# nerficg-project/nerficg

Measured on NVIDIA B200. Metric: nerf_train_rays_per_s, higher is better.
Workload: dtype fp16 operands, fp32 accumulate (fp32 sampling/compositing/optimizer)

## Files before the change

include/nerf_b200.h:

```cpp
#ifndef NERF_B200_H
#define NERF_B200_H

#include <stddef.h>
#include <stdint.h>

#ifdef __cplusplus
extern "C" {
#endif

#define NERF_ABI_VERSION 1

#define NERF_N_PARAM_TENSORS 24
#define NERF_TILE 128

int nerf_abi_version(void);
const char* nerf_last_error(void);
int nerf_device_check(int device);

int nerf_param_layout(int64_t* offsets , int64_t* sizes , int64_t* total);

int nerf_sample_stratified(float* z, const float* u, int n_rays, int n_samples, float near_plane, float far_plane,
                           void* stream);

int nerf_sample_importance(float* z_merged, float* z_fine, const float* z_coarse, const float* w_coarse, const float* u,
                           int n_rays, int n_coarse, int n_fine, void* stream);

int nerf_composite_forward(float* rgb, float* depth, float* alpha, float* weights, const float* z,
                           const float* rgbsigma, const float* dirs, const float* background, int n_rays, int n_samples,
                           void* stream);

int nerf_composite_backward(float* d_rgbsigma, const float* z, const float* rgbsigma, const float* dirs,
                            const float* background, const float* g_rgb, const float* g_depth, const float* g_alpha,
                            int n_rays, int n_samples, int relu_mask, float grad_scale, void* stream);

size_t nerf_mlp_packed_bytes(void);
int nerf_mlp_pack(void* packed, const float* params, int with_backward, void* stream);

size_t nerf_mlp_stash_bytes(int64_t n_samples);
int nerf_mlp_forward(float* rgbsigma, void* stash, const void* packed, const float* params, const float* origins,
                     const float* dirs, const float* viewdirs, const float* z, const float* noise, int n_rays,
                     int n_samples, void* stream);

size_t nerf_mlp_backward_workspace_bytes(int64_t n_samples);
int nerf_mlp_backward(float* grads, const float* d_rgbsigma, const float* rgbsigma, const void* stash, void* workspace,
                      const void* packed, const float* params, int n_rays, int n_samples, float grad_scale,
                      void* stream);

int nerf_mlp_backward_pipe(float* grads, const float* d_rgbsigma, const float* rgbsigma, const void* stash, void* workspace,
                           const void* packed, const float* params, int n_rays, int n_samples, float grad_scale, void* stream);
int nerf_mlp_backward_legacy(float* grads, const float* d_rgbsigma, const float* rgbsigma, const void* stash, void* workspace,
                             const void* packed, const float* params, int n_rays, int n_samples, float grad_scale, void* stream);
size_t nerf_mlp_backward_pipe_workspace_bytes(void);

int nerf_mlp_backward_dgrad(const float* d_rgbsigma, const float* rgbsigma, const void* stash, void* workspace,
                            const void* packed, const float* params, int n_rays, int n_samples, void* stream);
int nerf_mlp_backward_wgrad(float* grads, const void* stash, const void* workspace, int n_rays, int n_samples,
                            float grad_scale, void* stream);

int nerf_adam_tick(float* state, float beta1, float beta2, void* stream);
int nerf_adam_update(float* params, float* exp_avg, float* exp_avg_sq, const float* grads, const float* lr, const float* state,
                     float beta1, float beta2, float eps, int64_t n, void* stream);
int nerf_adam_update_ex(float* params, float* exp_avg, float* exp_avg_sq, float* grads, const float* lr, const float* state,
                        float beta1, float beta2, float eps, float grad_mult, int zero_grads, int64_t n, void* stream);

int nerf_loss_mse(float* loss, float* g_rgb, float* g_rgb_coarse, float* g_alpha, float* g_alpha_coarse, const float* rgb,
                  const float* rgb_coarse, const float* alpha, const float* alpha_coarse, const float* rgb_gt,
                  const float* alpha_gt, const float* background, int n_rays, float lambda_color, float lambda_alpha, void* stream);

int nerf_debug_set_timing(void* device_buffer);

int nerf_generate_rays(float* origin, float* direction, float* view_direction, const int64_t* pixel_ids, int64_t n_rays,
                       const double* c2w_host, int width, int height, double focal_x, double focal_y, double center_x,
                       double center_y, void* stream);
int nerf_gather_rays(float* origin_dst, float* direction_dst, float* view_direction_dst, float* rgb_dst, float* alpha_dst,
                     const float* origin_src, const float* direction_src, const float* view_direction_src, const float* rgb_src,
                     const float* alpha_src, const int64_t* ids, int64_t n_rays, void* stream);

int nerf_selftest_umma(float* d_out, const float* a, const float* b, int n, int k, int mode, void* stream);
int nerf_selftest_umma2(float* d_out, const float* a, const float* b, int n, int k, void* stream);
int nerf_selftest_umma2_mn(float* d_out, const float* a, const float* b, int n, int k, void* stream);
int nerf_selftest_tmem_read(unsigned long long* out, int n_warps, int mode, int iters, void* stream);

int nerf_selftest_umma2_rate(unsigned long long* out, int mn_major, int iters, void* stream);

int nerf_selftest_l2_stream(unsigned long long* out, void* window, uint32_t window_bytes, int mode, int iters, int n_ctas, void* stream);
int nerf_selftest_l2_stream_lsu(unsigned long long* out, void* window, uint32_t window_bytes, int mode, int iters, int n_ctas, int n_warps,
                                void* stream);

#ifdef __cplusplus
}
#endif
#endif
```

nerficg_b200/_lib.py:

```python
from __future__ import annotations

import ctypes
from ctypes import c_float, c_int, c_int64, c_size_t, c_void_p
from pathlib import Path

import torch

LIB_PATH = Path(__file__).resolve().parent / 'libnerf_b200.so'

_PROTOTYPES = {
    'nerf_abi_version': (c_int, []),
    'nerf_last_error': (ctypes.c_char_p, []),
    'nerf_device_check': (c_int, [c_int]),
    'nerf_param_layout': (c_int, [ctypes.POINTER(c_int64), ctypes.POINTER(c_int64), ctypes.POINTER(c_int64)]),
    'nerf_sample_stratified': (c_int, [c_void_p, c_void_p, c_int, c_int, c_float, c_float, c_void_p]),
    'nerf_sample_importance': (c_int, [c_void_p, c_void_p, c_void_p, c_void_p, c_void_p, c_int, c_int, c_int, c_void_p]),
    'nerf_composite_forward': (c_int, [c_void_p] * 8 + [c_int, c_int, c_void_p]),
    'nerf_composite_backward': (c_int, [c_void_p] * 8 + [c_int, c_int, c_int, c_float, c_void_p]),
    'nerf_mlp_packed_bytes': (c_size_t, []),
    'nerf_mlp_pack': (c_int, [c_void_p, c_void_p, c_int, c_void_p]),
    'nerf_mlp_stash_bytes': (c_size_t, [c_int64]),
    'nerf_mlp_forward': (c_int, [c_void_p] * 9 + [c_int, c_int, c_void_p]),
    'nerf_mlp_backward_workspace_bytes': (c_size_t, [c_int64]),
    'nerf_mlp_backward': (c_int, [c_void_p] * 7 + [c_int, c_int, c_float, c_void_p]),
    'nerf_mlp_backward_pipe': (c_int, [c_void_p] * 7 + [c_int, c_int, c_float, c_void_p]),
    'nerf_mlp_backward_legacy': (c_int, [c_void_p] * 7 + [c_int, c_int, c_float, c_void_p]),
    'nerf_mlp_backward_pipe_workspace_bytes': (c_size_t, []),
    'nerf_mlp_backward_dgrad': (c_int, [c_void_p] * 6 + [c_int, c_int, c_void_p]),
    'nerf_mlp_backward_wgrad': (c_int, [c_void_p] * 3 + [c_int, c_int, c_float, c_void_p]),
    'nerf_adam_tick': (c_int, [c_void_p, c_float, c_float, c_void_p]),
    'nerf_adam_update': (c_int, [c_void_p] * 6 + [c_float, c_float, c_float, c_int64, c_void_p]),
    'nerf_adam_update_ex': (c_int, [c_void_p] * 6 + [c_float, c_float, c_float, c_float, c_int, c_int64, c_void_p]),
    'nerf_generate_rays': (c_int, [c_void_p, c_void_p, c_void_p, c_void_p, c_int64, ctypes.POINTER(ctypes.c_double), c_int, c_int,
                                   ctypes.c_double, ctypes.c_double, ctypes.c_double, ctypes.c_double, c_void_p]),
    'nerf_gather_rays': (c_int, [c_void_p] * 11 + [c_int64, c_void_p]),
    'nerf_loss_mse': (c_int, [c_void_p] * 12 + [c_int, c_float, c_float, c_void_p]),
    'nerf_debug_set_timing': (c_int, [c_void_p]),
    'nerf_selftest_umma': (c_int, [c_void_p, c_void_p, c_void_p, c_int, c_int, c_int, c_void_p]),
    'nerf_selftest_umma2': (c_int, [c_void_p, c_void_p, c_void_p, c_int, c_int, c_void_p]),
    'nerf_selftest_umma2_mn': (c_int, [c_void_p, c_void_p, c_void_p, c_int, c_int, c_void_p]),
    'nerf_selftest_tmem_read': (c_int, [c_void_p, c_int, c_int, c_int, c_void_p]),
    'nerf_selftest_umma2_rate': (c_int, [c_void_p, c_int, c_int, c_void_p]),
    'nerf_selftest_l2_stream': (c_int, [c_void_p, c_void_p, ctypes.c_uint32, c_int, c_int, c_int, c_void_p]),
    'nerf_selftest_l2_stream_lsu': (c_int, [c_void_p, c_void_p, ctypes.c_uint32, c_int, c_int, c_int, c_int, c_void_p]),
}

EXPORTED_SYMBOLS = tuple(_PROTOTYPES)
_lib = None


class NativeLibraryError(RuntimeError):
    """The CUDA extension is missing, stale or running on an unsupported device."""


def load() -> ctypes.CDLL:
    global _lib
    if _lib is not None:
        return _lib
    if not LIB_PATH.exists():
        raise NativeLibraryError(
            f'{LIB_PATH} not found: build it with `python nerficg_b200/csrc/build.py` '
            '(there is no CPU or PyTorch fallback for the NeRF hot path)')
    lib = ctypes.CDLL(str(LIB_PATH))
    for name, (res, args) in _PROTOTYPES.items():
        try:
            fn = getattr(lib, name)
        except AttributeError as e:
            raise NativeLibraryError(f'{LIB_PATH} does not export {name}; rebuild the extension') from e
        fn.restype = res
        fn.argtypes = args
    if lib.nerf_abi_version() != 1:
        raise NativeLibraryError('ABI version mismatch; rebuild the extension')
    _lib = lib
    return lib


def last_error() -> str:
    return load().nerf_last_error().decode()


def check(rc: int, what: str) -> None:
    if rc != 0:
        raise NativeLibraryError(f'{what} failed ({rc}): {last_error()}')


_checked_devices: set[int] = set()


def require_device(t: torch.Tensor) -> None:
    if not t.is_cuda:
        raise NativeLibraryError('nerficg_b200 kernels need CUDA tensors on a B200 (sm_100); there is no CPU path')
    idx = t.device.index if t.device.index is not None else torch.cuda.current_device()
    if idx not in _checked_devices:
        check(load().nerf_device_check(idx), 'nerf_device_check')
        _checked_devices.add(idx)


def ptr(t: torch.Tensor | None) -> int | None:
    return None if t is None else t.data_ptr()


def stream_ptr() -> int:
    return torch.cuda.current_stream().cuda_stream


def param_layout() -> tuple[list[int], list[int], int]:
    off = (c_int64 * 24)()
    size = (c_int64 * 24)()
    total = c_int64()
    check(load().nerf_param_layout(off, size, ctypes.byref(total)), 'nerf_param_layout')
    return list(off), list(size), total.value
```

nerficg_b200/csrc/mlp_wgrad.cu:

```cuda
#include "common.cuh"
#include "mlp_layout.cuh"
#include "tc.cuh"
#include "../../include/nerf_b200.h"

namespace nerf {
using namespace tc;

namespace wg {
constexpr int kThreads = 256;
constexpr int kMaxStages = 8;
constexpr uint32_t kHalfPanel = 8192;
constexpr uint32_t kRingBytes = 24 * kHalfPanel;
constexpr uint32_t kOffBars = kRingBytes;
constexpr uint32_t kSmemBytes = kOffBars + 256 + 1024;
constexpr int kNumJobs = 13;

struct Seg {
  int16_t buf;
  int16_t region;
  int16_t panels;
  int16_t valid;
  int32_t out_col;
};
struct Job {
  Seg a;
  Seg b[2];
  int64_t w_off;
  int32_t ld;
  int64_t bias_off;
  int32_t head;
  int32_t ctas;
};

using L = ParamLayout;
constexpr Seg seg(int buf, int region, int panels, int valid, int out_col) { return Seg{(int16_t)buf, (int16_t)region, (int16_t)panels, (int16_t)valid, out_col}; }
constexpr Seg none() { return Seg{0, 0, 0, 0, 0}; }
constexpr int gl(int l) { return kGradL7 + (7 - l); }
constexpr int hx(int l) { return kStashH0 + l; }

__constant__ Job c_jobs[kNumJobs] = {
    {seg(0, gl(1), 4, 256, 0), {seg(1, hx(0), 4, 256, 0), none()}, L::hidden_w(1), 256, L::hidden_b(1), 0, 13},
    {seg(0, gl(2), 4, 256, 0), {seg(1, hx(1), 4, 256, 0), none()}, L::hidden_w(2), 256, L::hidden_b(2), 0, 13},
    {seg(0, gl(3), 4, 256, 0), {seg(1, hx(2), 4, 256, 0), none()}, L::hidden_w(3), 256, L::hidden_b(3), 0, 13},
    {seg(0, gl(4), 4, 256, 0), {seg(1, hx(3), 4, 256, 0), none()}, L::hidden_w(4), 256, L::hidden_b(4), 0, 13},
    {seg(0, gl(5), 4, 256, 0), {seg(1, hx(4), 4, 256, 0), none()}, L::kW5, 319, L::kB5, 0, 13},
    {seg(0, gl(6), 4, 256, 0), {seg(1, hx(5), 4, 256, 0), none()}, L::hidden_w(6), 256, L::hidden_b(6), 0, 13},
    {seg(0, gl(7), 4, 256, 0), {seg(1, hx(6), 4, 256, 0), none()}, L::hidden_w(7), 256, L::hidden_b(7), 0, 13},
    {seg(0, kGradF, 4, 256, 0), {seg(1, hx(7), 4, 256, 0), none()}, L::kWF, 256, L::kBF, 0, 13},
    {seg(0, gl(0), 4, 256, 0), {seg(1, kStashEnc, 1, 63, 0), none()}, L::kW0, 63, L::kB0, 0, 9},
    {seg(0, gl(5), 4, 256, 0), {seg(1, kStashEnc, 1, 63, 256), none()}, L::kW5, 319, -1, 0, 8},
    {seg(0, kGradC0, 2, 128, 0), {seg(1, kStashF, 4, 256, 0), seg(1, kStashDir, 1, 27, 256)}, L::kWC0, 283, L::kBC0, 0, 12},
    {seg(1, kStashG, 2, 128, 0), {seg(0, kGradHead, 1, 4, 0), none()}, L::kWC1, 128, L::kBC1, 1, 6},
    {seg(1, hx(7), 4, 256, 0), {seg(0, kGradHead, 1, 4, 0), none()}, L::kWS, 256, L::kBS, 2, 9},
};
constexpr int kNumResidualJobs = 4;
__constant__ Job c_jobs_res[kNumResidualJobs] = {
    {seg(0, gl(0), 4, 256, 0), {seg(1, kStashEnc, 1, 63, 0), none()}, L::kW0, 63, L::kB0, 0, 37},
    {seg(0, gl(5), 4, 256, 0), {seg(1, kStashEnc, 1, 63, 256), none()}, L::kW5, 319, -1, 0, 37},
    {seg(0, kGradC0, 2, 128, 0), {seg(1, kStashF, 4, 256, 0), seg(1, kStashDir, 1, 27, 256)}, L::kWC0, 283, L::kBC0, 0, 52},
    {seg(1, kStashG, 2, 128, 0), {seg(0, kGradHead, 1, 4, 0), none()}, L::kWC1, 128, L::kBC1, 1, 22},
};
}

__global__ void __launch_bounds__(wg::kThreads, 1) mlp_wgrad_kernel(float* __restrict__ grads, const uint8_t* __restrict__ stash,
                                                                     const uint8_t* __restrict__ gstash, int n_tiles, float inv_scale,
                                                                     int residual) {
  using namespace wg;
  const Job* __restrict__ table = residual ? c_jobs_res : c_jobs;
  const int n_jobs = residual ? kNumResidualJobs : kNumJobs;
  int job_idx = 0, part = (int)blockIdx.x;
  while (job_idx < n_jobs && part >= table[job_idx].ctas) part -= table[job_idx++].ctas;
  if (job_idx >= n_jobs) return;
  const Job& job = table[job_idx];
  const int parts = job.ctas;
  const int tile_lo = (int)((int64_t)n_tiles * part / parts), tile_hi = (int)((int64_t)n_tiles * (part + 1) / parts);
  const int n_steps = 2 * (tile_hi - tile_lo);
  if (n_steps <= 0) return;

  extern __shared__ uint8_t smem_raw[];
  const uint32_t smem_base = (smem_u32(smem_raw) + 1023u) & ~1023u;
  const uint32_t bars = smem_base + kOffBars;
  const uint32_t bar_full = bars, bar_empty = bars + 8 * kMaxStages, bar_done = bars + 16 * kMaxStages, tmem_slot = bar_done + 8;
  const uint32_t kStageBytes = (uint32_t)(job.a.panels + job.b[0].panels + job.b[1].panels) * kHalfPanel;
  const int kStages = (int)(kRingBytes / kStageBytes) < kMaxStages ? (int)(kRingBytes / kStageBytes) : kMaxStages;
  const int warp = threadIdx.x >> 5, lane = threadIdx.x & 31;
  if (threadIdx.x == 0) {
    for (int i = 0; i < kMaxStages; ++i) {
      mbar_init(bar_full + 8 * i, 1);
      mbar_init(bar_empty + 8 * i, 2);
    }
    mbar_init(bar_done, 1);
    fence_barrier_init();
  }
  if (warp == 2) {
    tmem_alloc(tmem_slot, 512);
    tmem_relinquish();
  }
  tc_fence_before();
  __syncthreads();
  tc_fence_after();
  uint32_t tmem_base;
  asm volatile("ld.shared.b32 %0, [%1];" : "=r"(tmem_base) : "r"(tmem_slot));

  const uint64_t nt = (uint64_t)n_tiles;
  const int na = job.a.panels;
  const int nb0 = job.b[0].panels, nb1 = job.b[1].panels;
  const int halves = na / 2;
  const int n_total = 64 * (nb0 + nb1);

  auto region_ptr = [&](const Seg& s, int tile) -> const uint8_t* {
    return s.buf == 0 ? gstash + grad_region_offset(s.region, nt) + (uint64_t)tile * grad_region_tile_bytes(s.region)
                      : stash + stash_region_offset(s.region, nt) + (uint64_t)tile * stash_region_tile_bytes(s.region);
  };

  if (warp == 0) {
    if (lane == 0) {
      uint32_t stage = 0, phase = 0;
      const uint64_t stream_policy = l2_evict_first();
      const Seg* segs[3] = {&job.a, &job.b[0], &job.b[1]};
      const uint8_t* cur[3];
      uint32_t tile_stride[3];
      int panels[3];
      for (int s = 0; s < 3; ++s) {
        panels[s] = segs[s]->panels;
        cur[s] = region_ptr(*segs[s], tile_lo);
        tile_stride[s] = segs[s]->buf == 0 ? grad_region_tile_bytes(segs[s]->region) : stash_region_tile_bytes(segs[s]->region);
      }
      const uint32_t stage_bytes = (uint32_t)(na + nb0 + nb1) * kHalfPanel;
      for (int step = 0; step < n_steps; ++step) {
        const uint32_t half_off = (step & 1) * kHalfPanel;
        mbar_wait(bar_empty + 8 * stage, phase ^ 1);
        mbar_arrive_expect_tx(bar_full + 8 * stage, stage_bytes);
        uint32_t dst = smem_base + stage * kStageBytes;
#pragma unroll
        for (int s = 0; s < 3; ++s) {
          const uint8_t* src = cur[s] + half_off;
          for (int pp = 0; pp < panels[s]; ++pp) {
            bulk_g2s_hint(dst, src, kHalfPanel, bar_full + 8 * stage, stream_policy);
            dst += kHalfPanel;
            src += kPanelBytes128;
          }
          if (step & 1) cur[s] += tile_stride[s];
        }
        if (++stage == kStages) {
          stage = 0;
          phase ^= 1;
        }
      }
    }
  } else if (warp == 1) {
    if (lane == 0) {
      uint32_t stage = 0, phase = 0;
      const uint32_t idesc_b0 = make_idesc(128, 64 * nb0, kF16, kF16, 1, 1);
      const uint32_t idesc_b1 = make_idesc(128, 64, kF16, kF16, 1, 1);
      for (int step = 0; step < n_steps; ++step) {
        mbar_wait(bar_full + 8 * stage, phase);
        tc_fence_after();
        const uint32_t sa = smem_base + stage * kStageBytes;
        const uint32_t sb0 = sa + na * kHalfPanel, sb1 = sb0 + nb0 * kHalfPanel;
        for (int hm = 0; hm < halves; ++hm) {
          const uint32_t d0 = tmem_base + hm * n_total;
          for (int ks = 0; ks < 4; ++ks) {
            const uint64_t da = desc_mnmajor(sa + hm * 2 * kHalfPanel, ks, kHalfPanel);
            umma(d0, da, desc_mnmajor(sb0, ks, kHalfPanel), idesc_b0, (step | ks) != 0);
            if (nb1 > 0) umma(d0 + 64 * nb0, da, desc_mnmajor(sb1, ks, kHalfPanel), idesc_b1, (step | ks) != 0);
          }
        }
        umma_commit(bar_empty + 8 * stage);
        if (++stage == kStages) {
          stage = 0;
          phase ^= 1;
        }
      }
      umma_commit(bar_done);
    }
  } else if (warp >= 4) {
    const int t = threadIdx.x - 128;
    const bool head = job.head != 0;
    const int bias_cols = head ? 4 : (job.bias_off >= 0 ? 64 * na : 0);
    const uint32_t bias_seg_off = head ? na * kHalfPanel : 0;
    float s0 = 0.f, s1 = 0.f;
    uint32_t stage = 0, phase = 0;
    for (int step = 0; step < n_steps; ++step) {
      mbar_wait(bar_full + 8 * stage, phase);
      if (2 * t < bias_cols) {
        const int c = 2 * t;
        const uint32_t base = smem_base + stage * kStageBytes + bias_seg_off + (c >> 6) * kHalfPanel;
#pragma unroll 8
        for (int r = 0; r < 64; ++r) {
          uint32_t w;
          asm volatile("ld.shared.b32 %0, [%1];" : "=r"(w) : "r"(base + panel_offset(r, c & 63)));
          const float2 f = __half22float2(*reinterpret_cast<__half2*>(&w));
          s0 += f.x;
          s1 += f.y;
        }
      }
      named_bar_sync(1, 128);
      if (t == 0) mbar_arrive(bar_empty + 8 * stage);
      if (++stage == kStages) {
        stage = 0;
        phase ^= 1;
      }
    }
    if (2 * t < bias_cols) {
      if (!head) {
        atomicAdd(grads + job.bias_off + 2 * t, s0 * inv_scale);
        atomicAdd(grads + job.bias_off + 2 * t + 1, s1 * inv_scale);
      } else if (job.head == 1) {
        if (t == 0) {
          atomicAdd(grads + job.bias_off + 0, s0 * inv_scale);
          atomicAdd(grads + job.bias_off + 1, s1 * inv_scale);
        } else {
          atomicAdd(grads + job.bias_off + 2, s0 * inv_scale);
        }
      } else if (t == 1) {
        atomicAdd(grads + job.bias_off, s1 * inv_scale);
      }
    }
    mbar_wait(bar_done, 0);
    tc_fence_after();
    const int wq = warp & 3;
    const int n_local = wq * 32 + lane;
    for (int hm = 0; hm < halves; ++hm) {
      const int n = hm * 128 + n_local;
      const uint32_t t_row = tmem_base + hm * n_total + (static_cast<uint32_t>(wq * 32) << 16);
      if (head) {
        uint32_t v[32];
        tmem_ld32(t_row, v);
        tmem_ld_wait();
        if (job.head == 1) {
#pragma unroll
          for (int j = 0; j < 3; ++j) atomicAdd(grads + job.w_off + j * 128 + n, __uint_as_float(v[j]) * inv_scale);
        } else {
          atomicAdd(grads + job.w_off + n, __uint_as_float(v[3]) * inv_scale);
        }
        continue;
      }
      float* wrow = grads + job.w_off + (int64_t)n * job.ld;
      for (int s = 0; s < 2; ++s) {
        const Seg& sg = job.b[s];
        if (sg.panels == 0) continue;
        const int col_base = s == 0 ? 0 : 64 * nb0;
        for (int c0 = 0; c0 < 64 * sg.panels; c0 += 32) {
          if (c0 >= sg.valid) break;
          uint32_t v[32];
          tmem_ld32(t_row + col_base + c0, v);
          tmem_ld_wait();
#pragma unroll
          for (int j = 0; j < 32; ++j)
            if (c0 + j < sg.valid) atomicAdd(wrow + sg.out_col + c0 + j, __uint_as_float(v[j]) * inv_scale);
        }
      }
    }
  }
  tc_fence_before();
  __syncthreads();
  if (warp == 2) tmem_dealloc(tmem_base, 512);
}

static int launch_wgrad_table(float* grads, const uint8_t* stash, const uint8_t* gstash, int n_tiles, float inv_scale, int residual, cudaStream_t stream);

int launch_wgrad(float* grads, const uint8_t* stash, const uint8_t* gstash, int n_tiles, float inv_scale, cudaStream_t stream) {
  return launch_wgrad_table(grads, stash, gstash, n_tiles, inv_scale, 0, stream);
}
int launch_wgrad_residual(float* grads, const uint8_t* stash, const uint8_t* gstash, int n_tiles, float inv_scale, cudaStream_t stream) {
  return launch_wgrad_table(grads, stash, gstash, n_tiles, inv_scale, 1, stream);
}

static int launch_wgrad_table(float* grads, const uint8_t* stash, const uint8_t* gstash, int n_tiles, float inv_scale, int residual, cudaStream_t stream) {
  static bool attr_set_dev[64] = {};
    int dev__ = 0;
    cudaGetDevice(&dev__);
    bool& attr_set = attr_set_dev[dev__ & 63];
  if (!attr_set) {
    cudaError_t e = cudaFuncSetAttribute(mlp_wgrad_kernel, cudaFuncAttributeMaxDynamicSharedMemorySize, (int)wg::kSmemBytes);
    NERF_CHECK_ARG(e == cudaSuccess, "mlp_backward: cudaFuncSetAttribute(wgrad) failed: %s", cudaGetErrorString(e));
    attr_set = true;
  }
  mlp_wgrad_kernel<<<kNumSMs, wg::kThreads, wg::kSmemBytes, stream>>>(grads, stash, gstash, n_tiles, inv_scale, residual);
  NERF_CHECK_LAUNCH("mlp_wgrad_kernel");
  return 0;
}

}
```

nerficg_b200/csrc/tc.cuh:

```cuda
#pragma once
#include <cuda_bf16.h>
#include <cuda_fp16.h>
#include <cstdint>

namespace nerf {
namespace tc {

constexpr uint32_t kPanelCols = 64;
constexpr uint32_t kPanelRowBytes = 128;
constexpr uint32_t kAtomBytes = 1024;

__host__ __device__ __forceinline__ uint32_t panel_offset(uint32_t row, uint32_t col) {
  return (row >> 3) * kAtomBytes + (row & 7) * kPanelRowBytes + ((((col >> 3) ^ (row & 7)) & 7) << 4) + ((col & 7) << 1);
}
__host__ __device__ __forceinline__ uint32_t panel_chunk_offset(uint32_t row, uint32_t chunk) {
  return (row >> 3) * kAtomBytes + (row & 7) * kPanelRowBytes + (((chunk ^ (row & 7)) & 7) << 4);
}

__device__ __forceinline__ uint32_t smem_u32(const void* p) { return static_cast<uint32_t>(__cvta_generic_to_shared(p)); }

__device__ __forceinline__ void mbar_init(uint32_t bar, uint32_t count) {
  asm volatile("mbarrier.init.shared::cta.b64 [%0], %1;" ::"r"(bar), "r"(count));
}
__device__ __forceinline__ void fence_barrier_init() { asm volatile("fence.mbarrier_init.release.cluster;" ::: "memory"); }
__device__ __forceinline__ void mbar_arrive(uint32_t bar) {
  asm volatile("mbarrier.arrive.shared::cta.b64 _, [%0];" ::"r"(bar) : "memory");
}
__device__ __forceinline__ void mbar_arrive_expect_tx(uint32_t bar, uint32_t bytes) {
  asm volatile("mbarrier.arrive.expect_tx.shared::cta.b64 _, [%0], %1;" ::"r"(bar), "r"(bytes) : "memory");
}
__device__ __forceinline__ bool mbar_try_wait(uint32_t bar, uint32_t parity) {
  uint32_t ok;
  asm volatile(
      "{\n\t.reg .pred p;\n\t"
      "mbarrier.try_wait.parity.shared::cta.b64 p, [%1], %2;\n\t"
      "selp.u32 %0, 1, 0, p;\n\t}"
      : "=r"(ok)
      : "r"(bar), "r"(parity)
      : "memory");
  return ok != 0;
}
__device__ __forceinline__ void mbar_wait(uint32_t bar, uint32_t parity) {
  while (!mbar_try_wait(bar, parity)) {
  }
}

__device__ __forceinline__ void fence_proxy_async_smem() { asm volatile("fence.proxy.async.shared::cta;" ::: "memory"); }

__device__ __forceinline__ void bulk_g2s(uint32_t dst_smem, const void* src, uint32_t bytes, uint32_t bar) {
  asm volatile("cp.async.bulk.shared::cluster.global.mbarrier::complete_tx::bytes [%0], [%1], %2, [%3];" ::"r"(dst_smem),
               "l"(src), "r"(bytes), "r"(bar)
               : "memory");
}
__device__ __forceinline__ void bulk_s2g(void* dst, uint32_t src_smem, uint32_t bytes) {
  asm volatile("cp.async.bulk.global.shared::cta.bulk_group [%0], [%1], %2;" ::"l"(dst), "r"(src_smem), "r"(bytes) : "memory");
}
__device__ __forceinline__ uint64_t l2_evict_first() {
  uint64_t p;
  asm volatile("createpolicy.fractional.L2::evict_first.b64 %0, 1.0;" : "=l"(p));
  return p;
}
__device__ __forceinline__ uint64_t l2_evict_last() {
  uint64_t p;
  asm volatile("createpolicy.fractional.L2::evict_last.b64 %0, 1.0;" : "=l"(p));
  return p;
}
__device__ __forceinline__ void bulk_g2s_hint(uint32_t dst_smem, const void* src, uint32_t bytes, uint32_t bar, uint64_t policy) {
  asm volatile("cp.async.bulk.shared::cluster.global.mbarrier::complete_tx::bytes.L2::cache_hint [%0], [%1], %2, [%3], %4;" ::"r"(dst_smem),
               "l"(src), "r"(bytes), "r"(bar), "l"(policy)
               : "memory");
}
__device__ __forceinline__ void bulk_s2g_hint(void* dst, uint32_t src_smem, uint32_t bytes, uint64_t policy) {
  asm volatile("cp.async.bulk.global.shared::cta.bulk_group.L2::cache_hint [%0], [%1], %2, %3;" ::"l"(dst), "r"(src_smem), "r"(bytes),
               "l"(policy)
               : "memory");
}
__device__ __forceinline__ void cp_async16(uint32_t dst_smem, const void* src) {
  asm volatile("cp.async.cg.shared.global [%0], [%1], 16;" ::"r"(dst_smem), "l"(src) : "memory");
}
__device__ __forceinline__ void cp_async_mbar_arrive_noinc(uint32_t bar) {
  asm volatile("cp.async.mbarrier.arrive.noinc.shared::cta.b64 [%0];" ::"r"(bar) : "memory");
}
__device__ __forceinline__ void cp_async_commit() { asm volatile("cp.async.commit_group;" ::: "memory"); }
template <int N>
__device__ __forceinline__ void cp_async_wait() {
  asm volatile("cp.async.wait_group %0;" ::"n"(N) : "memory");
}
__device__ __forceinline__ void bulk_commit() { asm volatile("cp.async.bulk.commit_group;" ::: "memory"); }
template <int N>
__device__ __forceinline__ void bulk_wait_read() {
  asm volatile("cp.async.bulk.wait_group.read %0;" ::"n"(N) : "memory");
}
template <int N>
__device__ __forceinline__ void bulk_wait_all() {
  asm volatile("cp.async.bulk.wait_group %0;" ::"n"(N) : "memory");
}

__device__ __forceinline__ void tmem_alloc(uint32_t dst_smem, uint32_t ncols) {
  asm volatile("tcgen05.alloc.cta_group::1.sync.aligned.shared::cta.b32 [%0], %1;" ::"r"(dst_smem), "r"(ncols) : "memory");
}
__device__ __forceinline__ void tmem_relinquish() { asm volatile("tcgen05.relinquish_alloc_permit.cta_group::1.sync.aligned;" ::: "memory"); }
__device__ __forceinline__ void tmem_dealloc(uint32_t taddr, uint32_t ncols) {
  asm volatile("tcgen05.dealloc.cta_group::1.sync.aligned.b32 %0, %1;" ::"r"(taddr), "r"(ncols) : "memory");
}
__device__ __forceinline__ void tc_fence_before() { asm volatile("tcgen05.fence::before_thread_sync;" ::: "memory"); }
__device__ __forceinline__ void tc_fence_after() { asm volatile("tcgen05.fence::after_thread_sync;" ::: "memory"); }
__device__ __forceinline__ void tmem_ld_wait() { asm volatile("tcgen05.wait::ld.sync.aligned;" ::: "memory"); }

__device__ __forceinline__ void tmem_ld32(uint32_t taddr, uint32_t (&r)[32]) {
  asm volatile(
      "tcgen05.ld.sync.aligned.32x32b.x32.b32 "
      "{%0, %1, %2, %3, %4, %5, %6, %7, %8, %9, %10, %11, %12, %13, %14, %15, "
      "%16, %17, %18, %19, %20, %21, %22, %23, %24, %25, %26, %27, %28, %29, %30, %31}, [%32];"
      : "=r"(r[0]), "=r"(r[1]), "=r"(r[2]), "=r"(r[3]), "=r"(r[4]), "=r"(r[5]), "=r"(r[6]), "=r"(r[7]), "=r"(r[8]),
        "=r"(r[9]), "=r"(r[10]), "=r"(r[11]), "=r"(r[12]), "=r"(r[13]), "=r"(r[14]), "=r"(r[15]), "=r"(r[16]),
        "=r"(r[17]), "=r"(r[18]), "=r"(r[19]), "=r"(r[20]), "=r"(r[21]), "=r"(r[22]), "=r"(r[23]), "=r"(r[24]),
        "=r"(r[25]), "=r"(r[26]), "=r"(r[27]), "=r"(r[28]), "=r"(r[29]), "=r"(r[30]), "=r"(r[31])
      : "r"(taddr)
      : "memory");
}

__device__ __forceinline__ void tmem_ld_wait32(uint32_t (&r)[32]) {
  asm volatile("tcgen05.wait::ld.sync.aligned;"
               : "+r"(r[0]), "+r"(r[1]), "+r"(r[2]), "+r"(r[3]), "+r"(r[4]), "+r"(r[5]), "+r"(r[6]), "+r"(r[7]), "+r"(r[8]),
                 "+r"(r[9]), "+r"(r[10]), "+r"(r[11]), "+r"(r[12]), "+r"(r[13]), "+r"(r[14]), "+r"(r[15]), "+r"(r[16]),
                 "+r"(r[17]), "+r"(r[18]), "+r"(r[19]), "+r"(r[20]), "+r"(r[21]), "+r"(r[22]), "+r"(r[23]), "+r"(r[24]),
                 "+r"(r[25]), "+r"(r[26]), "+r"(r[27]), "+r"(r[28]), "+r"(r[29]), "+r"(r[30]), "+r"(r[31])
               :
               : "memory");
}

__device__ __forceinline__ void tmem_ld16(uint32_t taddr, uint32_t (&r)[16]) {
  asm volatile(
      "tcgen05.ld.sync.aligned.32x32b.x16.b32 "
      "{%0, %1, %2, %3, %4, %5, %6, %7, %8, %9, %10, %11, %12, %13, %14, %15}, [%16];"
      : "=r"(r[0]), "=r"(r[1]), "=r"(r[2]), "=r"(r[3]), "=r"(r[4]), "=r"(r[5]), "=r"(r[6]), "=r"(r[7]), "=r"(r[8]),
        "=r"(r[9]), "=r"(r[10]), "=r"(r[11]), "=r"(r[12]), "=r"(r[13]), "=r"(r[14]), "=r"(r[15])
      : "r"(taddr)
      : "memory");
}
__device__ __forceinline__ void tmem_ld_wait16(uint32_t (&r)[16]) {
  asm volatile("tcgen05.wait::ld.sync.aligned;"
               : "+r"(r[0]), "+r"(r[1]), "+r"(r[2]), "+r"(r[3]), "+r"(r[4]), "+r"(r[5]), "+r"(r[6]), "+r"(r[7]), "+r"(r[8]),
                 "+r"(r[9]), "+r"(r[10]), "+r"(r[11]), "+r"(r[12]), "+r"(r[13]), "+r"(r[14]), "+r"(r[15])
               :
               : "memory");
}

template <int N>
__device__ __forceinline__ void setmaxnreg_inc() {
  asm volatile("setmaxnreg.inc.sync.aligned.u32 %0;" ::"n"(N));
}
template <int N>
__device__ __forceinline__ void setmaxnreg_dec() {
  asm volatile("setmaxnreg.dec.sync.aligned.u32 %0;" ::"n"(N));
}

__device__ __forceinline__ uint64_t make_smem_desc(uint32_t smem_addr, uint32_t lbo_bytes, uint32_t sbo_bytes) {
  uint64_t d = 0;
  d |= static_cast<uint64_t>((smem_addr & 0x3FFFFu) >> 4);
  d |= static_cast<uint64_t>((lbo_bytes >> 4) & 0x3FFFu) << 16;
  d |= static_cast<uint64_t>((sbo_bytes >> 4) & 0x3FFFu) << 32;
  d |= static_cast<uint64_t>(1) << 46;
  d |= static_cast<uint64_t>(2) << 61;
  return d;
}
__device__ __forceinline__ uint64_t desc_kmajor(uint32_t panel_smem, uint32_t kstep) {
  return make_smem_desc(panel_smem + kstep * 32u, 16u, kAtomBytes);
}
__device__ __forceinline__ uint64_t desc_mnmajor(uint32_t panel_smem, uint32_t kstep, uint32_t panel_stride) {
  return make_smem_desc(panel_smem + kstep * 2u * kAtomBytes, panel_stride, kAtomBytes);
}

enum : uint32_t { kF16 = 0, kBF16 = 1 };
__host__ __device__ constexpr uint32_t make_idesc(uint32_t m, uint32_t n, uint32_t a_fmt, uint32_t b_fmt, uint32_t a_mn_major,
                                                  uint32_t b_mn_major) {
  return (1u << 4) | (a_fmt << 7) | (b_fmt << 10) | (a_mn_major << 15) | (b_mn_major << 16) | ((n >> 3) << 17) |
         ((m >> 4) << 24);
}

__device__ __forceinline__ void umma(uint32_t d_tmem, uint64_t a_desc, uint64_t b_desc, uint32_t idesc, uint32_t accumulate) {
  asm volatile(
      "{\n\t.reg .pred p;\n\t"
      "setp.ne.b32 p, %4, 0;\n\t"
      "tcgen05.mma.cta_group::1.kind::f16 [%0], %1, %2, %3, p;\n\t}" ::"r"(d_tmem),
      "l"(a_desc), "l"(b_desc), "r"(idesc), "r"(accumulate)
      : "memory");
}
__device__ __forceinline__ void umma_commit(uint32_t bar) {
  asm volatile("tcgen05.commit.cta_group::1.mbarrier::arrive::one.shared::cluster.b64 [%0];" ::"r"(bar) : "memory");
}

__device__ __forceinline__ uint32_t cluster_ctarank() {
  uint32_t r;
  asm volatile("mov.u32 %0, %%cluster_ctarank;" : "=r"(r));
  return r;
}
__device__ __forceinline__ void cluster_sync_all() {
  asm volatile("barrier.cluster.arrive.release.aligned;\n\tbarrier.cluster.wait.acquire.aligned;" ::: "memory");
}
__device__ __forceinline__ uint32_t mapa(uint32_t smem_addr, uint32_t rank) {
  uint32_t r;
  asm volatile("mapa.shared::cluster.u32 %0, %1, %2;" : "=r"(r) : "r"(smem_addr), "r"(rank));
  return r;
}
__device__ __forceinline__ void mbar_arrive_cluster(uint32_t cluster_addr) {
  asm volatile("mbarrier.arrive.shared::cluster.b64 _, [%0];" ::"r"(cluster_addr) : "memory");
}
__device__ __forceinline__ void mbar_wait_cluster(uint32_t bar, uint32_t parity) { mbar_wait(bar, parity); }
__device__ __forceinline__ void tmem_alloc2(uint32_t dst_smem, uint32_t ncols) {
  asm volatile("tcgen05.alloc.cta_group::2.sync.aligned.shared::cta.b32 [%0], %1;" ::"r"(dst_smem), "r"(ncols) : "memory");
}
__device__ __forceinline__ void tmem_relinquish2() { asm volatile("tcgen05.relinquish_alloc_permit.cta_group::2.sync.aligned;" ::: "memory"); }
__device__ __forceinline__ void tmem_dealloc2(uint32_t taddr, uint32_t ncols) {
  asm volatile("tcgen05.dealloc.cta_group::2.sync.aligned.b32 %0, %1;" ::"r"(taddr), "r"(ncols) : "memory");
}
__device__ __forceinline__ void umma2(uint32_t d_tmem, uint64_t a_desc, uint64_t b_desc, uint32_t idesc, uint32_t accumulate) {
  asm volatile(
      "{\n\t.reg .pred p;\n\t"
      "setp.ne.b32 p, %4, 0;\n\t"
      "tcgen05.mma.cta_group::2.kind::f16 [%0], %1, %2, %3, p;\n\t}" ::"r"(d_tmem),
      "l"(a_desc), "l"(b_desc), "r"(idesc), "r"(accumulate)
      : "memory");
}
__device__ __forceinline__ void umma_commit2(uint32_t bar, uint16_t cta_mask) {
  asm volatile("tcgen05.commit.cta_group::2.mbarrier::arrive::one.shared::cluster.multicast::cluster.b64 [%0], %1;" ::"r"(bar),
               "h"(cta_mask)
               : "memory");
}

__device__ __forceinline__ uint32_t pack_half2(float a, float b) {
  __half2 h = __floats2half2_rn(a, b);
  return *reinterpret_cast<uint32_t*>(&h);
}
__device__ __forceinline__ uint32_t pack_bf162(float a, float b) {
  __nv_bfloat162 h = __floats2bfloat162_rn(a, b);
  return *reinterpret_cast<uint32_t*>(&h);
}
__device__ __forceinline__ uint32_t half2_gt0_mask(uint32_t w) {
  const __half2 z = __floats2half2_rn(0.f, 0.f);
  return __hgt2_mask(*reinterpret_cast<__half2*>(&w), z);
}
__device__ __forceinline__ uint32_t half2_relu(uint32_t w) {
  const __half2 r = __hmax2(*reinterpret_cast<__half2*>(&w), __floats2half2_rn(0.f, 0.f));
  return *reinterpret_cast<const uint32_t*>(&r);
}
__host__ __device__ __forceinline__ uint32_t relu_mask_bit(uint32_t j) { return (j >> 1) + ((j & 1u) << 4); }

__device__ __forceinline__ void st_shared_v4(uint32_t addr, uint32_t a, uint32_t b, uint32_t c, uint32_t d) {
  asm volatile("st.shared.v4.b32 [%0], {%1, %2, %3, %4};" ::"r"(addr), "r"(a), "r"(b), "r"(c), "r"(d) : "memory");
}
__device__ __forceinline__ void named_bar_sync(uint32_t id, uint32_t nthreads) {
  asm volatile("bar.sync %0, %1;" ::"r"(id), "r"(nthreads) : "memory");
}
__device__ __forceinline__ bool elect_one() {
  uint32_t pred;
  asm volatile(
      "{\n\t.reg .pred p;\n\t"
      "elect.sync _|p, 0xffffffff;\n\t"
      "selp.u32 %0, 1, 0, p;\n\t}"
      : "=r"(pred));
  return pred != 0;
}

}
}
```

Before: 845,500.

## Load wgrad operands with 3D TMA tensor maps in finer-grained pipeline steps

Replaces the per-panel 1D bulk copies in the weight-gradient kernel with one 3D tensor-map TMA load per operand segment per step, and splits each tile into 32-row steps instead of 64-row halves. The ring buffer and stage count grow, giving a deeper pipeline of smaller stages. Host-side tensor maps are encoded and cached per buffer pointer set. A probe entry point with a configurable grid is also added. The aim is to cut TMA issue overhead and improve load/MMA overlap, at the cost of more barrier traffic and smaller MMA K per step.

```diff
diff --git a/include/nerf_b200.h b/include/nerf_b200.h
--- a/include/nerf_b200.h
+++ b/include/nerf_b200.h
@@ -87,6 +87,9 @@
 int nerf_selftest_l2_stream_lsu(unsigned long long* out, void* window, uint32_t window_bytes, int mode, int iters, int n_ctas, int n_warps,
                                 void* stream);
 
+int nerf_mlp_wgrad_probe(float* grads, const void* stash, const void* workspace, int n_rays, int n_samples, int grid,
+                         uint64_t* bytes_out, void* stream);
+
 #ifdef __cplusplus
 }
 #endif
diff --git a/nerficg_b200/_lib.py b/nerficg_b200/_lib.py
--- a/nerficg_b200/_lib.py
+++ b/nerficg_b200/_lib.py
@@ -43,6 +43,7 @@
     'nerf_selftest_umma2_rate': (c_int, [c_void_p, c_int, c_int, c_void_p]),
     'nerf_selftest_l2_stream': (c_int, [c_void_p, c_void_p, ctypes.c_uint32, c_int, c_int, c_int, c_void_p]),
     'nerf_selftest_l2_stream_lsu': (c_int, [c_void_p, c_void_p, ctypes.c_uint32, c_int, c_int, c_int, c_int, c_void_p]),
+    'nerf_mlp_wgrad_probe': (c_int, [c_void_p] * 3 + [c_int, c_int, c_int, ctypes.POINTER(ctypes.c_uint64), c_void_p]),
 }
 
 EXPORTED_SYMBOLS = tuple(_PROTOTYPES)
diff --git a/nerficg_b200/csrc/mlp_wgrad.cu b/nerficg_b200/csrc/mlp_wgrad.cu
--- a/nerficg_b200/csrc/mlp_wgrad.cu
+++ b/nerficg_b200/csrc/mlp_wgrad.cu
@@ -1,3 +1,6 @@
+#include <cuda.h>
+#include <cudaTypedefs.h>
+#include <mutex>
 #include "common.cuh"
 #include "mlp_layout.cuh"
 #include "tc.cuh"
@@ -8,12 +11,23 @@
 
 namespace wg {
 constexpr int kThreads = 256;
-constexpr int kMaxStages = 8;
-constexpr uint32_t kHalfPanel = 8192;
-constexpr uint32_t kRingBytes = 24 * kHalfPanel;
+#ifndef NERF_WGRAD_STEP_ROWS
+#define NERF_WGRAD_STEP_ROWS 32
+#endif
+constexpr int kStepRows = NERF_WGRAD_STEP_ROWS;
+constexpr int kStepsPerTile = kTile / kStepRows;
+constexpr uint32_t kStepPanel = kStepRows * 128;
+constexpr int kMaxStages = 16;
+constexpr uint32_t kRingBytes = 56 * 4096;
 constexpr uint32_t kOffBars = kRingBytes;
-constexpr uint32_t kSmemBytes = kOffBars + 256 + 1024;
+constexpr uint32_t kSmemBytes = kOffBars + 512 + 1024;
+static_assert(kSmemBytes <= 232448, "shared memory budget exceeded");
+static_assert(kRingBytes % kStepPanel == 0 && kStepRows % 16 == 0, "step geometry");
 constexpr int kNumJobs = 13;
+struct Maps {
+  CUtensorMap m[2][3];
+};
+__host__ __device__ constexpr int depth_index(int panels) { return panels == 4 ? 2 : panels - 1; }
 
 struct Seg {
   int16_t buf;
@@ -62,26 +76,25 @@
 };
 }
 
-__global__ void __launch_bounds__(wg::kThreads, 1) mlp_wgrad_kernel(float* __restrict__ grads, const uint8_t* __restrict__ stash,
-                                                                     const uint8_t* __restrict__ gstash, int n_tiles, float inv_scale,
-                                                                     int residual) {
+__global__ void __launch_bounds__(wg::kThreads, 1) mlp_wgrad_kernel(float* __restrict__ grads, const __grid_constant__ wg::Maps maps,
+                                                                     int n_tiles, float inv_scale, int residual) {
   using namespace wg;
   const Job* __restrict__ table = residual ? c_jobs_res : c_jobs;
   const int n_jobs = residual ? kNumResidualJobs : kNumJobs;
-  int job_idx = 0, part = (int)blockIdx.x;
+  int job_idx = 0, part = (int)((int)blockIdx.x * kNumSMs / (int)gridDim.x);
   while (job_idx < n_jobs && part >= table[job_idx].ctas) part -= table[job_idx++].ctas;
   if (job_idx >= n_jobs) return;
   const Job& job = table[job_idx];
   const int parts = job.ctas;
   const int tile_lo = (int)((int64_t)n_tiles * part / parts), tile_hi = (int)((int64_t)n_tiles * (part + 1) / parts);
-  const int n_steps = 2 * (tile_hi - tile_lo);
+  const int n_steps = kStepsPerTile * (tile_hi - tile_lo);
   if (n_steps <= 0) return;
 
   extern __shared__ uint8_t smem_raw[];
   const uint32_t smem_base = (smem_u32(smem_raw) + 1023u) & ~1023u;
   const uint32_t bars = smem_base + kOffBars;
   const uint32_t bar_full = bars, bar_empty = bars + 8 * kMaxStages, bar_done = bars + 16 * kMaxStages, tmem_slot = bar_done + 8;
-  const uint32_t kStageBytes = (uint32_t)(job.a.panels + job.b[0].panels + job.b[1].panels) * kHalfPanel;
+  const uint32_t kStageBytes = (uint32_t)(job.a.panels + job.b[0].panels + job.b[1].panels) * kStepPanel;
   const int kStages = (int)(kRingBytes / kStageBytes) < kMaxStages ? (int)(kRingBytes / kStageBytes) : kMaxStages;
   const int warp = threadIdx.x >> 5, lane = threadIdx.x & 31;
   if (threadIdx.x == 0) {
@@ -108,39 +121,34 @@
   const int halves = na / 2;
   const int n_total = 64 * (nb0 + nb1);
 
-  auto region_ptr = [&](const Seg& s, int tile) -> const uint8_t* {
-    return s.buf == 0 ? gstash + grad_region_offset(s.region, nt) + (uint64_t)tile * grad_region_tile_bytes(s.region)
-                      : stash + stash_region_offset(s.region, nt) + (uint64_t)tile * stash_region_tile_bytes(s.region);
-  };
-
   if (warp == 0) {
     if (lane == 0) {
       uint32_t stage = 0, phase = 0;
       const uint64_t stream_policy = l2_evict_first();
       const Seg* segs[3] = {&job.a, &job.b[0], &job.b[1]};
-      const uint8_t* cur[3];
-      uint32_t tile_stride[3];
-      int panels[3];
+      const CUtensorMap* tmap[3];
+      int panel[3], tile_panels[3], panels[3];
       for (int s = 0; s < 3; ++s) {
-        panels[s] = segs[s]->panels;
-        cur[s] = region_ptr(*segs[s], tile_lo);
-        tile_stride[s] = segs[s]->buf == 0 ? grad_region_tile_bytes(segs[s]->region) : stash_region_tile_bytes(segs[s]->region);
-      }
-      const uint32_t stage_bytes = (uint32_t)(na + nb0 + nb1) * kHalfPanel;
+        const Seg& sg = *segs[s];
+        panels[s] = sg.panels;
+        tmap[s] = &maps.m[sg.buf][depth_index(sg.panels > 0 ? sg.panels : 1)];
+        const uint32_t tile_bytes = sg.buf == 0 ? grad_region_tile_bytes(sg.region) : stash_region_tile_bytes(sg.region);
+        const uint64_t off = (sg.buf == 0 ? grad_region_offset(sg.region, nt) : stash_region_offset(sg.region, nt)) + (uint64_t)tile_lo * tile_bytes;
+        panel[s] = (int)(off / kPanelBytes128);
+        tile_panels[s] = (int)(tile_bytes / kPanelBytes128);
+      }
+      const uint32_t stage_bytes = (uint32_t)(na + nb0 + nb1) * kStepPanel;
       for (int step = 0; step < n_steps; ++step) {
-        const uint32_t half_off = (step & 1) * kHalfPanel;
+        const int sub = step % kStepsPerTile;
+        const int row0 = sub * kStepRows;
         mbar_wait(bar_empty + 8 * stage, phase ^ 1);
         mbar_arrive_expect_tx(bar_full + 8 * stage, stage_bytes);
         uint32_t dst = smem_base + stage * kStageBytes;
 #pragma unroll
         for (int s = 0; s < 3; ++s) {
-          const uint8_t* src = cur[s] + half_off;
-          for (int pp = 0; pp < panels[s]; ++pp) {
-            bulk_g2s_hint(dst, src, kHalfPanel, bar_full + 8 * stage, stream_policy);
-            dst += kHalfPanel;
-            src += kPanelBytes128;
-          }
-          if (step & 1) cur[s] += tile_stride[s];
+          if (panels[s] > 0) tma_g2s_3d_hint(dst, tmap[s], 0, row0, panel[s], bar_full + 8 * stage, stream_policy);
+          dst += panels[s] * kStepPanel;
+          if (sub == kStepsPerTile - 1) panel[s] += tile_panels[s];
         }
         if (++stage == kStages) {
           stage = 0;
@@ -157,13 +165,13 @@
         mbar_wait(bar_full + 8 * stage, phase);
         tc_fence_after();
         const uint32_t sa = smem_base + stage * kStageBytes;
-        const uint32_t sb0 = sa + na * kHalfPanel, sb1 = sb0 + nb0 * kHalfPanel;
+        const uint32_t sb0 = sa + na * kStepPanel, sb1 = sb0 + nb0 * kStepPanel;
         for (int hm = 0; hm < halves; ++hm) {
           const uint32_t d0 = tmem_base + hm * n_total;
-          for (int ks = 0; ks < 4; ++ks) {
-            const uint64_t da = desc_mnmajor(sa + hm * 2 * kHalfPanel, ks, kHalfPanel);
-            umma(d0, da, desc_mnmajor(sb0, ks, kHalfPanel), idesc_b0, (step | ks) != 0);
-            if (nb1 > 0) umma(d0 + 64 * nb0, da, desc_mnmajor(sb1, ks, kHalfPanel), idesc_b1, (step | ks) != 0);
+          for (int ks = 0; ks < kStepRows / 16; ++ks) {
+            const uint64_t da = desc_mnmajor(sa + hm * 2 * kStepPanel, ks, kStepPanel);
+            umma(d0, da, desc_mnmajor(sb0, ks, kStepPanel), idesc_b0, (step | ks) != 0);
+            if (nb1 > 0) umma(d0 + 64 * nb0, da, desc_mnmajor(sb1, ks, kStepPanel), idesc_b1, (step | ks) != 0);
           }
         }
         umma_commit(bar_empty + 8 * stage);
@@ -178,16 +186,16 @@
     const int t = threadIdx.x - 128;
     const bool head = job.head != 0;
     const int bias_cols = head ? 4 : (job.bias_off >= 0 ? 64 * na : 0);
-    const uint32_t bias_seg_off = head ? na * kHalfPanel : 0;
+    const uint32_t bias_seg_off = head ? na * kStepPanel : 0;
     float s0 = 0.f, s1 = 0.f;
     uint32_t stage = 0, phase = 0;
     for (int step = 0; step < n_steps; ++step) {
       mbar_wait(bar_full + 8 * stage, phase);
       if (2 * t < bias_cols) {
         const int c = 2 * t;
-        const uint32_t base = smem_base + stage * kStageBytes + bias_seg_off + (c >> 6) * kHalfPanel;
+        const uint32_t base = smem_base + stage * kStageBytes + bias_seg_off + (c >> 6) * kStepPanel;
 #pragma unroll 8
-        for (int r = 0; r < 64; ++r) {
+        for (int r = 0; r < kStepRows; ++r) {
           uint32_t w;
           asm volatile("ld.shared.b32 %0, [%1];" : "=r"(w) : "r"(base + panel_offset(r, c & 63)));
           const float2 f = __half22float2(*reinterpret_cast<__half2*>(&w));
@@ -258,28 +266,117 @@
   if (warp == 2) tmem_dealloc(tmem_base, 512);
 }
 
-static int launch_wgrad_table(float* grads, const uint8_t* stash, const uint8_t* gstash, int n_tiles, float inv_scale, int residual, cudaStream_t stream);
-
-int launch_wgrad(float* grads, const uint8_t* stash, const uint8_t* gstash, int n_tiles, float inv_scale, cudaStream_t stream) {
-  return launch_wgrad_table(grads, stash, gstash, n_tiles, inv_scale, 0, stream);
-}
-int launch_wgrad_residual(float* grads, const uint8_t* stash, const uint8_t* gstash, int n_tiles, float inv_scale, cudaStream_t stream) {
-  return launch_wgrad_table(grads, stash, gstash, n_tiles, inv_scale, 1, stream);
-}
-
-static int launch_wgrad_table(float* grads, const uint8_t* stash, const uint8_t* gstash, int n_tiles, float inv_scale, int residual, cudaStream_t stream) {
+namespace {
+PFN_cuTensorMapEncodeTiled_v12000 tensor_map_encoder() {
+  static const PFN_cuTensorMapEncodeTiled_v12000 fn = [] {
+    void* f = nullptr;
+    cudaDriverEntryPointQueryResult q = cudaDriverEntryPointSymbolNotFound;
+    if (cudaGetDriverEntryPointByVersion("cuTensorMapEncodeTiled", &f, 12000, cudaEnableDefault, &q) != cudaSuccess ||
+        q != cudaDriverEntryPointSuccess)
+      f = nullptr;
+    return reinterpret_cast<PFN_cuTensorMapEncodeTiled_v12000>(f);
+  }();
+  return fn;
+}
+
+bool encode_panel_map(PFN_cuTensorMapEncodeTiled_v12000 encode, CUtensorMap* map, const void* base, uint64_t n_panels, uint32_t depth) {
+  const cuuint64_t dims[3] = {tc::kPanelRowBytes, (cuuint64_t)kTile, n_panels};
+  const cuuint64_t strides[2] = {tc::kPanelRowBytes, kPanelBytes128};
+  const cuuint32_t box[3] = {tc::kPanelRowBytes, (cuuint32_t)wg::kStepRows, depth};
+  const cuuint32_t elem_strides[3] = {1, 1, 1};
+  return encode(map, CU_TENSOR_MAP_DATA_TYPE_UINT8, 3, const_cast<void*>(base), dims, strides, box, elem_strides, CU_TENSOR_MAP_INTERLEAVE_NONE,
+                CU_TENSOR_MAP_SWIZZLE_NONE, CU_TENSOR_MAP_L2_PROMOTION_L2_256B, CU_TENSOR_MAP_FLOAT_OOB_FILL_NONE) == CUDA_SUCCESS;
+}
+
+struct MapCacheEntry {
+  const void* stash = nullptr;
+  const void* gstash = nullptr;
+  int n_tiles = 0;
+  wg::Maps maps;
+};
+std::mutex g_map_mutex;
+MapCacheEntry g_map_cache[8];
+int g_map_next = 0;
+
+int wgrad_maps(wg::Maps* out, const uint8_t* stash, const uint8_t* gstash, int n_tiles) {
+  std::lock_guard<std::mutex> lock(g_map_mutex);
+  for (const MapCacheEntry& e : g_map_cache)
+    if (e.n_tiles == n_tiles && e.stash == stash && e.gstash == gstash) {
+      *out = e.maps;
+      return 0;
+    }
+  const PFN_cuTensorMapEncodeTiled_v12000 encode = tensor_map_encoder();
+  NERF_CHECK_ARG(encode != nullptr, "mlp_backward: cuTensorMapEncodeTiled is not available from the driver");
+  const uint64_t nt = (uint64_t)n_tiles;
+  const uint64_t panels[2] = {grad_tile_bytes_total() * nt / kPanelBytes128, stash_region_offset(kStashMask, nt) / kPanelBytes128};
+  const void* bases[2] = {gstash, stash};
+  MapCacheEntry& e = g_map_cache[g_map_next];
+  for (int b = 0; b < 2; ++b)
+    for (int d = 0; d < 3; ++d)
+      NERF_CHECK_ARG(encode_panel_map(encode, &e.maps.m[b][d], bases[b], panels[b], 1u << d),
+                     "mlp_backward: cuTensorMapEncodeTiled failed (buffer %d, %d panels)", b, 1 << d);
+  e.stash = stash;
+  e.gstash = gstash;
+  e.n_tiles = n_tiles;
+  g_map_next = (g_map_next + 1) % 8;
+  *out = e.maps;
+  return 0;
+}
+}
+
+static int launch_wgrad_table(float* grads, const uint8_t* stash, const uint8_t* gstash, int n_tiles, float inv_scale, int residual,
+                              int grid, cudaStream_t stream) {
+  if (n_tiles <= 0) return 0;
   static bool attr_set_dev[64] = {};
-    int dev__ = 0;
-    cudaGetDevice(&dev__);
-    bool& attr_set = attr_set_dev[dev__ & 63];
+  int dev__ = 0;
+  cudaGetDevice(&dev__);
+  bool& attr_set = attr_set_dev[dev__ & 63];
   if (!attr_set) {
     cudaError_t e = cudaFuncSetAttribute(mlp_wgrad_kernel, cudaFuncAttributeMaxDynamicSharedMemorySize, (int)wg::kSmemBytes);
     NERF_CHECK_ARG(e == cudaSuccess, "mlp_backward: cudaFuncSetAttribute(wgrad) failed: %s", cudaGetErrorString(e));
     attr_set = true;
   }
-  mlp_wgrad_kernel<<<kNumSMs, wg::kThreads, wg::kSmemBytes, stream>>>(grads, stash, gstash, n_tiles, inv_scale, residual);
+  wg::Maps maps;
+  if (int rc = wgrad_maps(&maps, stash, gstash, n_tiles)) return rc;
+  mlp_wgrad_kernel<<<grid, wg::kThreads, wg::kSmemBytes, stream>>>(grads, maps, n_tiles, inv_scale, residual);
   NERF_CHECK_LAUNCH("mlp_wgrad_kernel");
   return 0;
 }
 
-}
+int launch_wgrad(float* grads, const uint8_t* stash, const uint8_t* gstash, int n_tiles, float inv_scale, cudaStream_t stream) {
+  return launch_wgrad_table(grads, stash, gstash, n_tiles, inv_scale, 0, kNumSMs, stream);
+}
+int launch_wgrad_residual(float* grads, const uint8_t* stash, const uint8_t* gstash, int n_tiles, float inv_scale, cudaStream_t stream) {
+  return launch_wgrad_table(grads, stash, gstash, n_tiles, inv_scale, 1, kNumSMs, stream);
+}
+
+static uint64_t wgrad_grid_bytes(int n_tiles, int grid) {
+  wg::Job jobs[wg::kNumJobs];
+  if (cudaMemcpyFromSymbol(jobs, wg::c_jobs, sizeof(jobs)) != cudaSuccess) return 0;
+  uint64_t bytes = 0;
+  for (int b = 0; b < grid; ++b) {
+    int j = 0, part = b * kNumSMs / grid;
+    while (j < wg::kNumJobs && part >= jobs[j].ctas) part -= jobs[j++].ctas;
+    if (j >= wg::kNumJobs) continue;
+    const int64_t lo = (int64_t)n_tiles * part / jobs[j].ctas, hi = (int64_t)n_tiles * (part + 1) / jobs[j].ctas;
+    bytes += (uint64_t)(hi - lo) * (jobs[j].a.panels + jobs[j].b[0].panels + jobs[j].b[1].panels) * kPanelBytes128;
+  }
+  return bytes;
+}
+
+}
+
+extern "C" int nerf_mlp_wgrad_probe(float* grads, const void* stash, const void* workspace, int n_rays, int n_samples, int grid,
+                                    uint64_t* bytes_out, void* stream) {
+  using namespace nerf;
+  NERF_CHECK_ARG(grads && stash && workspace && bytes_out, "mlp_wgrad_probe: null pointer");
+  NERF_CHECK_ARG(grid >= 1 && grid <= kNumSMs, "mlp_wgrad_probe: grid must be in 1..%d", kNumSMs);
+  NERF_CHECK_ARG(((reinterpret_cast<uintptr_t>(stash) | reinterpret_cast<uintptr_t>(workspace)) & 127) == 0,
+                 "mlp_wgrad_probe: stash and workspace must be 128-byte aligned");
+  const int64_t n_evals = (int64_t)n_rays * n_samples;
+  NERF_CHECK_ARG(n_evals > 0 && n_evals < (int64_t(1) << 31) - kTile, "mlp_wgrad_probe: bad sample count");
+  const int n_tiles = (int)((n_evals + kTile - 1) / kTile);
+  *bytes_out = wgrad_grid_bytes(n_tiles, grid);
+  return launch_wgrad_table(grads, static_cast<const uint8_t*>(stash), static_cast<const uint8_t*>(workspace), n_tiles, 1.f, 0, grid,
+                            static_cast<cudaStream_t>(stream));
+}
diff --git a/nerficg_b200/csrc/tc.cuh b/nerficg_b200/csrc/tc.cuh
--- a/nerficg_b200/csrc/tc.cuh
+++ b/nerficg_b200/csrc/tc.cuh
@@ -69,6 +69,12 @@
   asm volatile("cp.async.bulk.shared::cluster.global.mbarrier::complete_tx::bytes.L2::cache_hint [%0], [%1], %2, [%3], %4;" ::"r"(dst_smem),
                "l"(src), "r"(bytes), "r"(bar), "l"(policy)
                : "memory");
+}
+__device__ __forceinline__ void tma_g2s_3d_hint(uint32_t dst_smem, const void* tmap, int x, int y, int z, uint32_t bar, uint64_t policy) {
+  asm volatile(
+      "cp.async.bulk.tensor.3d.shared::cluster.global.tile.mbarrier::complete_tx::bytes.L2::cache_hint [%0], [%1, {%2, %3, %4}], [%5], %6;" ::"r"(dst_smem),
+      "l"(tmap), "r"(x), "r"(y), "r"(z), "r"(bar), "l"(policy)
+      : "memory");
 }
 __device__ __forceinline__ void bulk_s2g_hint(void* dst, uint32_t src_smem, uint32_t bytes, uint64_t policy) {
   asm volatile("cp.async.bulk.global.shared::cta.bulk_group.L2::cache_hint [%0], [%1], %2, %3;" ::"l"(dst), "r"(src_smem), "r"(bytes),
```

Measured after the change: 786,500 (median of 6 runs). -7.0%, worse.
